# ska-telescope/ska-sdp-distributed-fourier-transform

Hardware: AMD Instinct MI355X
Metric: facet_to_subgrid_contributions_per_s (higher is better)
Workload: dtype complex64 (f32 arithmetic)

## Files before the change

### include/swiftly_hip.h

```cpp
#ifndef SWIFTLY_HIP_H
#define SWIFTLY_HIP_H

#include <stddef.h>
#include <stdint.h>

#ifdef __cplusplus
extern "C" {
#endif

typedef struct swiftly_hip swiftly_hip_t;

enum { SWIFTLY_C64 = 0, SWIFTLY_C128 = 1 };
enum {
    SWIFTLY_OK = 0,
    SWIFTLY_ERR_PARAM = 1,
    SWIFTLY_ERR_UNSUPPORTED = 2,
    SWIFTLY_ERR_HIP = 3
};

const char* swiftly_hip_last_error(void);
int swiftly_hip_version(void);
int swiftly_hip_device_count(void);
const char* swiftly_hip_build_id(void);

// ... 185 lines not shown
                                               const int64_t* sub_off0s, void* g_out, int64_t g_facet_stride,
                                               int64_t g_sub_stride, const int64_t* g_offsets,
                                               const int64_t* g_facet_strides, void* stream);
int swiftly_hip_k3_one_launch(int on);

int swiftly_hip_sum_finish_facets(swiftly_hip_t* h, int dtype, const void* in, int64_t nfacets, int64_t in_facet_stride,
                                  int64_t in_sub_stride, int64_t in_row_stride, const int64_t* facet_off0s,
                                  const int64_t* facet_off1s, void* out, int64_t out_sub_stride, int64_t out_row_stride,
                                  const int64_t* subgrid_off1s, int64_t subgrid_size, const void* mask,
                                  int64_t mask_batch_stride, int64_t nsub, void* stream);

int swiftly_hip_wave_facet_side(swiftly_hip_t* h, int dtype, const void* bands, int64_t rows, int64_t band_row_stride,
                                int64_t band_facet_stride, int64_t nfacets, const int64_t* facet_off0s,
                                int64_t band_start, int64_t band_len, int64_t wave_off1, const int32_t* rowmap,
                                int64_t n_rows, void* q_work, int64_t q_facet_stride, int compute_q, int64_t nsub,
                                const int64_t* sub_off0s, void* g_out, int64_t g_facet_stride, int64_t g_sub_stride,
                                const int64_t* g_offsets, const int64_t* g_facet_strides, void* scratch,
                                int64_t scratch_bytes, void* stream);
int swiftly_hip_wave_subgrid_side(swiftly_hip_t* h, int dtype, const void* g, int64_t nfacets, int64_t g_facet_stride,
                                  int64_t g_sub_stride, const int64_t* facet_off0s, const int64_t* facet_off1s,
                                  int64_t nsub, const int64_t* sub_off0s, const int64_t* sub_off1s, int64_t subgrid_size,
                                  const void* mask0, int64_t mask0_bs, const void* mask1, int64_t mask1_bs,
                                  void* tmp_work, void* out, void* scratch, int64_t scratch_bytes, void* stream);

int swiftly_hip_wave_group_finish_pieces(swiftly_hip_t* h, int dtype, int64_t npieces, const void* const* q,
                                         const int64_t* q_facet_strides, const int32_t* const* rowmaps,
                                         const int64_t* n_rows, const int64_t* first, const int64_t* count,
                                         int64_t nfacets, const int64_t* facet_off0s, const int64_t* facet_off1s,
                                         int64_t nsub, const int64_t* sub_off0s, const int64_t* sub_off1s,
                                         int64_t subgrid_size, const void* mask0, int64_t mask0_bs, const void* mask1,
                                         int64_t mask1_bs, void* t_work, int64_t t_work_elems, void* out, int stages,
                                         void* stream);
int swiftly_hip_group_finish(int on);

int swiftly_hip_finish_axis1_rows(swiftly_hip_t* h, int dtype, const void* bands, int64_t rows, int64_t band_row_stride,
                                  int64_t band_facet_stride, int64_t nfacets, const int64_t* facet_off1s,
                                  int64_t band_start, int64_t band_len, int64_t wave_off1, void* out,
                                  int64_t out_row_stride, int64_t out_facet_stride, void* stream);
int swiftly_hip_wave_subgrid_side_placed(swiftly_hip_t* h, int dtype, const void* g, int64_t nfacets, int64_t g_facet_stride,
                                         int64_t g_sub_stride, const int64_t* facet_off0s, const int64_t* facet_off1s,
                                         int64_t nsub, const int64_t* sub_off0s, const int64_t* sub_off1s,
                                         int64_t subgrid_size, const void* mask0, int64_t mask0_bs, const void* mask1,
                                         int64_t mask1_bs, void* tmp_work, void* out, void* scratch, int64_t scratch_bytes,
                                         void* stream);

int swiftly_hip_prepare_facet_window_rows(swiftly_hip_t* h, int dtype, const void* in, int64_t rows, int64_t facet_size,
                                          int64_t in_row_stride, void* out, int64_t out_row_stride, int64_t facet_off,
                                          int64_t band_start, int64_t band_len, int64_t other_axis_size,
                                          int64_t other_axis_row0, const int32_t* window_starts, int64_t nwindows,
                                          int64_t out_window_stride, void* stream);
int swiftly_hip_split_prepare_facets(swiftly_hip_t* h, int dtype, const void* in, int64_t in_sub_stride,
                                     int64_t in_row_stride, int64_t subgrid_size, int64_t nsub,
                                     const int64_t* subgrid_off1s, int64_t nfacets, const int64_t* facet_off0s,
                                     const int64_t* facet_off1s, void* out, int64_t out_facet_stride,
                                     int64_t out_sub_stride, void* stream);

int swiftly_hip_wave_split_subgrids(swiftly_hip_t* h, int dtype, const void* subgrids, int64_t subgrid_size, int64_t nsub,
                                    const int64_t* subgrid_off0s, const int64_t* subgrid_off1s, int64_t nfacets,
                                    const int64_t* facet_off0s, const int64_t* facet_off1s, void* work,
                                    int64_t work_elems, void* out, int64_t out_facet_stride, int64_t out_sub_stride,
                                    void* stream);

int swiftly_hip_accumulate_facet_columns(swiftly_hip_t* h, int dtype, const void* parts, int64_t part_row_stride,
                                         int64_t nchunks, const int64_t* chunk_offsets,
                                         const int64_t* chunk_facet_strides, const int32_t* row_sources,
                                         int64_t nfacets, const int64_t* facet_off0s, int64_t facet_size,
// ... 51 lines not shown
```

### ska-sdp-distributed-fourier-transform_amd/csrc/group_finish.hip

```cpp
#include "swiftly_groupfinish.h"
#include "swiftly_launch.h"

namespace swf {

template <int LOGM, int LOGX>
static int launch_one_g(const GroupFinishArgs& a, int nbatch, int ngroups, hipStream_t s) {
    using S = GFGeo<LOGM, LOGX>;
    dim3 grid((unsigned)((a.ncols + 15) / 16), (unsigned)nbatch, (unsigned)ngroups);
    return launch_lds<group_finish_kernel<LOGM, LOGX>, S::LDS_BYTES>(grid, dim3(S::NT), s, a);
}

int launch_group_finish(int logm, int logx, const GroupFinishArgs& a, int nbatch, int ngroups, hipStream_t s) {
#define GF_CASE(M, XX) \
    if (logm == M && logx == XX) return launch_one_g<M, XX>(a, nbatch, ngroups, s);
    GF_PAIRS(GF_CASE)
#undef GF_CASE
    return -1;
}

}
```

### ska-sdp-distributed-fourier-transform_amd/csrc/swiftly_abi.hip

```cpp
#include <hip/hip_runtime.h>
#include "swiftly_abi_internal.h"

static thread_local std::string g_err;

int fail(int code, const char* fmt, ...) {
    char buf[512];
    va_list ap;
    va_start(ap, fmt);
    vsnprintf(buf, sizeof buf, fmt, ap);
    va_end(ap);
    g_err = buf;
    return code;
}

int launch_status(int e, const char* what, const char* negative) {
    if (!e) return 0;
    const char* text = (e < 0 && negative) ? negative : hipGetErrorString((hipError_t)e);
    if (what) return fail(SWIFTLY_ERR_HIP, "kernel launch failed (%s): %s", what, text);
    return fail(SWIFTLY_ERR_HIP, "kernel launch failed: %s", text);
}
int radix_launch_status(int e, int Q, const char* pass) {
    if (!e) return 0;
    char what[48]; snprintf(what, sizeof what, "radix-%d %s", Q, pass);
    return launch_status(e, what);
// ... 150 lines not shown
    }
    return n;
}

int swiftly_hip_create(swiftly_hip_t** out, int64_t N, int64_t yN, int64_t xM, double W, const double* pswf,
                       int device) {
    if (!out || !pswf) return fail(SWIFTLY_ERR_PARAM, "null argument");
    *out = nullptr;
    if (const std::string bad = check_sizes(N, yN, xM); !bad.empty()) return fail(SWIFTLY_ERR_PARAM, "%s", bad.c_str());
    int ndev = swiftly_hip_device_count();
    if (ndev <= 0) return fail(SWIFTLY_ERR_HIP, "no HIP device visible: the SwiFTly HIP backend has no CPU fallback");
    if (device < 0 || device >= ndev) return fail(SWIFTLY_ERR_PARAM, "invalid device %d", device);
    DeviceGuard guard(device);
    if (guard.rc) return fail(SWIFTLY_ERR_HIP, "hipSetDevice(%d): %s", device, hipGetErrorString((hipError_t)guard.rc));
    std::lock_guard<std::mutex> init_lock(g_init_mutex);
    if ((int)g_device_inited.size() < ndev) g_device_inited.resize(ndev, 0);
    if (!g_device_inited[device]) {
        int lds = 0;
        if (int rc = set_registered_kernel_attributes(&lds))
            return fail(SWIFTLY_ERR_HIP, "kernel attribute setup failed (%d bytes of LDS): %d", lds, rc);
        hipMemPool_t pool;
        if (hipDeviceGetDefaultMemPool(&pool, device) == hipSuccess) {
            uint64_t keep = UINT64_MAX;
            (void)hipMemPoolSetAttribute(pool, hipMemPoolAttrReleaseThreshold, &keep);
        }
        (void)hipGetLastError();
        g_device_inited[device] = 1;
    }
    swiftly_hip* h = new (std::nothrow) swiftly_hip();
    if (!h) return fail(SWIFTLY_ERR_HIP, "out of host memory");
    static_cast<Sizes&>(*h) = make_sizes(N, yN, xM);
    h->W = W;
    h->device = device;
    if (const char* e = getenv("SWIFTLY_COL_F64")) h->col_f64 = atoi(e) != 0;
    if (const char* e = getenv("SWIFTLY_COL_F64_STAGES")) h->col_f64_stages = atoi(e) & 7;
    std::vector<double> ip(yN);
    std::vector<float> ipf(yN);
    for (int64_t k = 0; k < yN; k++) {
        ip[k] = (k == 0 || pswf[k] == 0.0) ? 0.0 : 1.0 / pswf[k];
        ipf[k] = (float)ip[k];
    }
    const int64_t step = N / xM;
    std::vector<double> fn;
    for (int64_t k = (yN / 2) % step; k < yN; k += step) fn.push_back(pswf[k]);
    if ((int64_t)fn.size() != h->m) {
        delete h;
        return fail(SWIFTLY_ERR_PARAM, "internal: Fn length %zu != contribution size %lld", fn.size(), (long long)(xM * yN / N));
    }
    std::vector<float> fnf(fn.begin(), fn.end());
    int rc = 0;
    if (!rc) rc = upload(h, &h->invp_d, ip);
    if (!rc) rc = upload(h, &h->invp_f, ipf);
    if (!rc) rc = upload(h, &h->fn_d, fn);
    if (!rc) rc = upload(h, &h->fn_f, fnf);
    for (int l : {h->log_yN, h->log_xM, h->log_m})
        if (!rc && l >= 0) {
            rc = make_twiddles(h, l);
            if (!rc && l >= kTwoPassMinLog) rc = make_twiddles(h, l / 2);
            if (!rc && l >= kTwoPassMinLog) rc = make_twiddles(h, l - l / 2);
            if (!rc && l == 15) rc = make_twiddles(h, 14);
            if (!rc && l == 15) rc = make_twiddles(h, 13);
            if (!rc && (l == 16 || l == 14)) rc = make_twiddles(h, l - 1);
        }
    if (!rc && h->log_yN == 15) {
        rc = make_compact_twiddles(h, 14, 5);
        if (!rc) h->win4.twc = compact_twiddles(h, 14, 5);
// ... 1096 lines not shown
```

### ska-sdp-distributed-fourier-transform_amd/csrc/swiftly_abi_internal.h

```cpp
#pragma once

#include <algorithm>
#include <cmath>
#include <cstdarg>
#include <cstdio>
#include <cstdlib>
#include <cstring>
#include <map>
#include <atomic>
#include <mutex>
#include <new>
#include <string>
#include <vector>

#include "../../include/swiftly_hip.h"
#include "swiftly_colpass.h"
#include "swiftly_geometry.h"
#include "swiftly_launch.h"
#include "swiftly_rowpass.h"
#include "swiftly_sumfinish.h"
#include "swiftly_rows.h"
#include "swiftly_rowslong.h"
#include "swiftly_bluestein.h"
#include "swiftly_mixed.h"
// ... 9 lines not shown
              "the complex128 backward band stays inside the double twiddle tables, the complex128 column passes and the long-row kernels");

int fail(int code, const char* fmt, ...);
#define HIP_TRY(expr)                                                                      \
    do {                                                                                   \
        hipError_t e_ = (expr);                                                            \
        if (e_ != hipSuccess) return fail(SWIFTLY_ERR_HIP, "%s: %s", #expr, hipGetErrorString(e_)); \
    } while (0)
int launch_status(int e, const char* what = nullptr, const char* negative = nullptr);
int radix_launch_status(int e, int Q, const char* pass = "pass");

struct ScratchLease {
    void* p = nullptr; bool own = false; hipStream_t st = nullptr;
    int acquire(void* ws, size_t ws_bytes, size_t need, hipStream_t stream, const char* what) {
        own = !(ws && ws_bytes >= need);
        st = stream;
        p = ws;
        if (!own) return 0;
        const hipError_t e = hipMallocAsync(&p, need, st);
        if (e == hipSuccess) return 0;
        own = false;
        return fail(SWIFTLY_ERR_HIP, "%s: %s", what, hipGetErrorString(e));
    }
    int release(int rc) {
        const hipError_t e = own ? hipFreeAsync(p, st) : hipSuccess;
        own = false;
        return (!rc && e != hipSuccess) ? fail(SWIFTLY_ERR_HIP, "hipFreeAsync: %s", hipGetErrorString(e)) : rc;
    }
};

struct swiftly_hip : Sizes {
    double W;
    int device;
    float* invp_f = nullptr;
    double* invp_d = nullptr;
    float* fn_f = nullptr;
    double* fn_d = nullptr;
    std::map<int, cx<float>*> tw_f;
    std::map<int, cx<double>*> tw_d;
    std::map<std::pair<int, int>, cx<float>*> twc_f;
    struct Blu {
        int logL = 0;
        cx<float>* chirp_f = nullptr;
        cx<float>* spec_f = nullptr;
        cx<double>* chirp_d = nullptr;
        cx<double>* spec_d = nullptr;
    };
    std::map<int64_t, Blu> blu;
    struct Mixed {
        int Q = 0, logM = 0;
        cx<float>* tw_f = nullptr;
        cx<double>* tw_d = nullptr;
    };
    std::map<int64_t, Mixed> mixed;
    std::vector<void*> allocs;
    int col_f64 = 0;
    int col_f64_stages = 7;
    hipStream_t chunk_st[2] = {nullptr, nullptr};
    std::mutex chunk_mu;
    std::atomic<void*> ws_plain_pending{nullptr};
    Win4Cache win4;
};

template <typename R>
inline MixedArgs<R> mixed_args(const swiftly_hip::Mixed& mx, int64_t n) {
    MixedArgs<R> X;
// ... 196 lines not shown
```

### ska-sdp-distributed-fourier-transform_amd/csrc/swiftly_abi_pipeline.hip

```cpp
#include "swiftly_abi_internal.h"
#include "swiftly_groupfinish.h"

__global__ void mark_columns_kernel(unsigned char* __restrict__ touched, int m, int rot, int base, int yN, int band_start,
                                    int band_len) {
    const int col = blockIdx.x * blockDim.x + threadIdx.x;
    if (col >= m) return;
    int scol = base + ((col + rot) & (m - 1));
    if (scol >= yN) scol -= yN;
    int d = scol - band_start;
    if (d < 0) d += yN;
    if (d < band_len) touched[d] = 1;
}
template <typename R>
__global__ void zero_untouched_kernel(cx<R>* __restrict__ band, const unsigned char* __restrict__ touched, long long rows,
                                      long long pitch, int band_len) {
    const int d = blockIdx.x * blockDim.x + threadIdx.x;
    if (d >= band_len || touched[d]) return;
    for (long long r = blockIdx.y; r < rows; r += gridDim.y) band[r * pitch + d] = cx<R>{(R)0, (R)0};
}


extern "C" {

int swiftly_hip_sum_finish_rows(swiftly_hip_t* h, int dtype, const void* in, int64_t ngroups, int64_t in_group_stride,
// ... 385 lines not shown
        }
    }
    return 0;
}

static int check_window_pieces(const swiftly_hip_t* h, const char* who, int64_t npieces, const void* const* q,
                               const int64_t* q_facet_strides, const int64_t* n_rows, const int64_t* first,
                               const int64_t* count) {
    if (npieces < 0 || npieces > 2) return fail(SWIFTLY_ERR_PARAM, "%s: 0..2 pieces, got %lld", who, (long long)npieces);
    const int64_t m = h->m;
    int64_t covered = 0;
    for (int64_t i = 0; i < npieces; i++) {
        if (count[i] < 0 || first[i] < 0 || first[i] + count[i] > m || first[i] % 16 || count[i] % 16)
            return fail(SWIFTLY_ERR_PARAM, "%s: piece %lld = [%lld, +%lld) must be multiples of 16 "
                        "inside [0, %lld)", who, (long long)i, (long long)first[i], (long long)count[i], (long long)m);
        if (count[i] && (!q[i] || n_rows[i] <= 0 || n_rows[i] > h->yN || q_facet_strides[i] < n_rows[i] * m))
            return fail(SWIFTLY_ERR_PARAM, "bad row count %lld / facet stride %lld", (long long)n_rows[i], (long long)q_facet_strides[i]);
        covered += count[i];
    }
    if (npieces == 2 && count[0] && count[1] && first[0] < first[1] + count[1] && first[1] < first[0] + count[0])
        return fail(SWIFTLY_ERR_PARAM, "%s: the pieces overlap", who);
    if (covered != m) return fail(SWIFTLY_ERR_PARAM, "%s: the pieces hold %lld of %lld positions", who, (long long)covered, (long long)m);
    return 0;
}

static void window_piece_roles(int64_t m, int64_t npieces, const int64_t* first, const int64_t* count, int* a, int* b) {
    *a = *b = -1;
    for (int64_t i = 0; i < npieces; i++)
        if (count[i]) *(first[i] == 0 && count[i] < m ? b : a) = (int)i;
}

static std::atomic<int> g_k3_one_launch{getenv("SWIFTLY_K3_ONE_LAUNCH") ? atoi(getenv("SWIFTLY_K3_ONE_LAUNCH")) != 0 : 1};
static std::atomic<int> g_group_finish{getenv("SWIFTLY_GROUP_FINISH") ? atoi(getenv("SWIFTLY_GROUP_FINISH")) != 0 : 1};

extern "C" {
int swiftly_hip_k3_one_launch(int on) {
    return on < 0 ? g_k3_one_launch.load() : g_k3_one_launch.exchange(on ? 1 : 0);
}

int swiftly_hip_transform_contributions(swiftly_hip_t* h, int dtype, const void* in, int layout, int64_t in_row_stride,
                                        int64_t in_facet_stride, int64_t in_sub_stride, const int32_t* in_rowmap,
                                        int64_t band_start, int64_t band_len, int64_t nfacets,
                                        const int64_t* facet_off0s, int64_t nsub, const int64_t* subgrid_offs,
                                        void* out, int64_t out_facet_stride, int64_t out_sub_stride, void* stream) {
    if (!h) return fail(SWIFTLY_ERR_PARAM, "null argument");
    DeviceGuard device_guard_(h->device);
    return transform_contributions_impl(h, dtype, in, layout, in_row_stride, in_facet_stride, in_sub_stride, in_rowmap,
                                        band_start, band_len, nfacets, facet_off0s, nsub, subgrid_offs, out,
                                        out_facet_stride, out_sub_stride, nullptr, nullptr, stream);
}

int swiftly_hip_transform_contributions_pieces(swiftly_hip_t* h, int dtype, int64_t npieces, const void* const* q,
                                               const int64_t* q_facet_strides, const int32_t* const* rowmaps,
                                               const int64_t* n_rows, const int64_t* first, const int64_t* count,
                                               int64_t nfacets, const int64_t* facet_off0s, int64_t nsub,
                                               const int64_t* sub_off0s, void* g_out, int64_t g_facet_stride,
                                               int64_t g_sub_stride, const int64_t* g_offsets,
                                               const int64_t* g_facet_strides, void* stream) {
    if (!h || !q || !q_facet_strides || !rowmaps || !n_rows || !first || !count || !g_out || !facet_off0s || !sub_off0s)
        return fail(SWIFTLY_ERR_PARAM, "null argument");
    if (!g_offsets != !g_facet_strides) return fail(SWIFTLY_ERR_PARAM, "g_offsets and g_facet_strides go together");
    if (int rc = check_window_pieces(h, "transform_contributions_pieces", npieces, q, q_facet_strides, n_rows, first, count)) return rc;
    DeviceGuard device_guard_(h->device);
    const int64_t m = h->m;
    int a, b;
    window_piece_roles(m, npieces, first, count, &a, &b);
// ... 245 lines not shown
                                    tmp_work, xM * xA, xA, sub_off1s, subgrid_size, mask1, mask1_bs, nsub, placed, stream);
    if (rc) return rc;
    CallWorkspace call_ws(scratch, scratch ? (size_t)scratch_bytes : 0);
    return swiftly_hip_finish_subgrid_batch(h, dtype, tmp_work, xA, 1, xA, out, 1, xA, 0, subgrid_size, mask0, nsub,
                                            xM * xA, xA * xA, sub_off0s, mask0 ? mask0_bs : 0, stream);
}

int swiftly_hip_wave_subgrid_side(swiftly_hip_t* h, int dtype, const void* g, int64_t nfacets, int64_t g_facet_stride,
                                  int64_t g_sub_stride, const int64_t* facet_off0s, const int64_t* facet_off1s,
                                  int64_t nsub, const int64_t* sub_off0s, const int64_t* sub_off1s, int64_t subgrid_size,
                                  const void* mask0, int64_t mask0_bs, const void* mask1, int64_t mask1_bs,
                                  void* tmp_work, void* out, void* scratch, int64_t scratch_bytes, void* stream) {
    return wave_subgrid_side_impl(h, dtype, g, nfacets, g_facet_stride, g_sub_stride, facet_off0s, facet_off1s, nsub, sub_off0s,
                                  sub_off1s, subgrid_size, mask0, mask0_bs, mask1, mask1_bs, tmp_work, out, scratch, scratch_bytes,
                                  0, stream);
}

int swiftly_hip_wave_subgrid_side_placed(swiftly_hip_t* h, int dtype, const void* g, int64_t nfacets, int64_t g_facet_stride,
                                         int64_t g_sub_stride, const int64_t* facet_off0s, const int64_t* facet_off1s,
                                         int64_t nsub, const int64_t* sub_off0s, const int64_t* sub_off1s,
                                         int64_t subgrid_size, const void* mask0, int64_t mask0_bs, const void* mask1,
                                         int64_t mask1_bs, void* tmp_work, void* out, void* scratch, int64_t scratch_bytes,
                                         void* stream) {
    return wave_subgrid_side_impl(h, dtype, g, nfacets, g_facet_stride, g_sub_stride, facet_off0s, facet_off1s, nsub, sub_off0s,
                                  sub_off1s, subgrid_size, mask0, mask0_bs, mask1, mask1_bs, tmp_work, out, scratch, scratch_bytes,
                                  1, stream);
}


int swiftly_hip_group_finish(int on) {
    return on < 0 ? g_group_finish.load() : g_group_finish.exchange(on ? 1 : 0);
}

int swiftly_hip_wave_group_finish_pieces(swiftly_hip_t* h, int dtype, int64_t npieces, const void* const* q,
                                         const int64_t* q_facet_strides, const int32_t* const* rowmaps,
                                         const int64_t* n_rows, const int64_t* first, const int64_t* count,
                                         int64_t nfacets, const int64_t* facet_off0s, const int64_t* facet_off1s,
                                         int64_t nsub, const int64_t* sub_off0s, const int64_t* sub_off1s,
                                         int64_t subgrid_size, const void* mask0, int64_t mask0_bs, const void* mask1,
                                         int64_t mask1_bs, void* t_work, int64_t t_work_elems, void* out, int stages,
                                         void* stream) {
    if (!h || !q || !q_facet_strides || !rowmaps || !n_rows || !first || !count || !t_work || !facet_off0s || !facet_off1s ||
        !sub_off0s || !sub_off1s || (!out && (stages & 2)))
        return fail(SWIFTLY_ERR_PARAM, "null argument");
    if (stages < 1 || stages > 3) return fail(SWIFTLY_ERR_PARAM, "wave_group_finish_pieces: stages must be 1, 2 or 3");
    CHECK_SUBGRID_SIZE();
    if (nfacets <= 0) return fail(SWIFTLY_ERR_UNSUPPORTED, "wave_group_finish_pieces: 1..%d facets supported", kGroupFinishMaxFacets);
    if (const std::string why = why_not_group_finish(*h, dtype, nfacets); !why.empty())
        return fail(SWIFTLY_ERR_UNSUPPORTED, "wave_group_finish_pieces: %s", why.c_str());
    if (h->col_f64)
        return fail(SWIFTLY_ERR_UNSUPPORTED, "wave_group_finish_pieces: float32 column arithmetic only (column precision is 64)");
    if (int rc = check_window_pieces(h, "wave_group_finish_pieces", npieces, q, q_facet_strides, n_rows, first, count)) return rc;
    if (nsub <= 0) return 0;
    DeviceGuard device_guard_(h->device);
    const int m = (int)h->m, xM = (int)h->xM, xA = (int)subgrid_size, yN = (int)h->yN, ratio = xM / m;
    CHECK_OFFSETS_32(offsets_fit_32(yN, m, yN));

    SumFinishFacetArgs r;
    std::memset(&r, 0, sizeof r);
    fill_facet_groups(r, h, nfacets, facet_off0s, facet_off1s);
    const int ngroups = r.ngroups;
    if (t_work_elems < (int64_t)ngroups * nsub * xM * m)
        return fail(SWIFTLY_ERR_PARAM, "t_work holds %lld elements, %lld needed", (long long)t_work_elems,
                    (long long)((int64_t)ngroups * nsub * xM * m));
    GroupFinishArgs a;
    std::memset(&a, 0, sizeof a);
// ... 17 lines not shown
    a.tw_x = twiddles<float>(h, h->log_xM);
    if (!a.fn || !a.tw_m || !a.tw_x) return fail(SWIFTLY_ERR_HIP, "internal: missing twiddle tables");
    a.mask_bs = mask0 ? mask0_bs : 0;

    for (int g = 0; g < ngroups; g++) {
        r.gstart[g] = g * ratio;
        for (int c = 0; c < ratio; c++) {
            r.fidx[g * ratio + c] = (int)((int64_t)g * nsub * ratio + c);
            r.base0[g * ratio + c] = c * m;
        }
    }
    r.gstart[ngroups] = ngroups * ratio;
    r.nfacets = ngroups * ratio;
    r.in_fs = (long long)m * m; r.in_bs = (long long)xM * m; r.in_rs = m;
    r.out_bs = (long long)xA * xA; r.out_rs = xA;
    r.nrows = xA;
    r.xA = xA;
    fill_group_rounds(r, h);
    r.mask_bs = mask1 ? mask1_bs : 0;
    if (int rc = fill_sum_finish_tables(h, false, &r.fn, &r.tw_m, &r.tw_x, &r.twc_m, &r.twc_x)) return rc;

    static_assert(kGroupFinishMaxBatch == kSumFinishMaxBatch, "one batch loop");
    for (int64_t b0 = 0; b0 < nsub; b0 += kGroupFinishMaxBatch) {
        const int nb = (int)std::min<int64_t>(kGroupFinishMaxBatch, nsub - b0);
        if (stages & 1) {
            a.out = (cx<float>*)t_work + b0 * a.out_bs;
            a.mask = mask0 ? (const float*)mask0 + b0 * mask0_bs : nullptr;
            for (int b = 0; b < nb; b++) {
                const Window w = window_of(*h, sub_off0s[b0 + b]);
                a.lda[b] = w.rot;
                a.ldc[b] = w.base;
                a.st_a[b] = subgrid_in_padded_subgrid(*h, xA, sub_off0s[b0 + b]).a;
            }
            if (int rc = launch_status(launch_group_finish(h->log_m, h->log_xM, a, nb, ngroups, (hipStream_t)stream), "group_finish",
                                       "no instance"))
                return rc;
        }
        if (stages & 2) {
            r.in = (const cx<float>*)t_work + b0 * r.in_bs;
            r.out = (cx<float>*)out + b0 * r.out_bs;
            r.mask = mask1 ? (const float*)mask1 + b0 * mask1_bs : nullptr;
            for (int b = 0; b < nb; b++) r.st_a[b] = subgrid_in_padded_subgrid(*h, xA, sub_off1s[b0 + b]).a;
            if (int rc = launch_status(launch_sum_finish_facets(h->log_m, h->log_xM, r, nb, (hipStream_t)stream))) return rc;
        }
    }
    return 0;
}

int swiftly_hip_accumulate_facet_columns(swiftly_hip_t* h, int dtype, const void* parts, int64_t part_row_stride,
                                         int64_t nchunks, const int64_t* chunk_offsets,
                                         const int64_t* chunk_facet_strides, const int32_t* row_sources,
                                         int64_t nfacets, const int64_t* facet_off0s, int64_t facet_size,
                                         const void* masks, int64_t subgrid_off1, void* bands, int64_t band_row_stride,
                                         int64_t band_facet_stride, int64_t band_start, int64_t band_len,
                                         unsigned char* touched, void* workspace, int64_t workspace_bytes,
                                         void* stream) {
    if (!h || !parts || !bands || !chunk_offsets || !chunk_facet_strides || !row_sources || !facet_off0s)
        return fail(SWIFTLY_ERR_PARAM, "null argument");
    DeviceGuard device_guard_(h->device);
    const bool c128 = dtype == SWIFTLY_C128;
    CHECK_DTYPE();
    CHECK_FACET_SIZE();
    const int yN = (int)h->yN, m = (int)h->m;
    const swiftly_hip::Mixed* mx = nullptr;
    if (h->log_yN < 0) {
        auto it = h->mixed.find(h->yN);
        if (it != h->mixed.end() && it->second.tw_f && !band_is_split(h)) mx = &it->second;
    }
    if (const std::string why = why_not_backward_band(*h, dtype, true); !why.empty())
// ... 112 lines not shown
```

### ska-sdp-distributed-fourier-transform_amd/csrc/swiftly_groupfinish.h

```cpp
#pragma once
#include "swiftly_caps.h"
#include "swiftly_colpass.h"

namespace swf {

constexpr int kGroupFinishMaxBatch = 64;

struct GroupFinishArgs {
    const cx<float>* in_a;
    const cx<float>* in_b;
    long long in_fs_a, in_fs_b;
    const int* rowmap_a;
    const int* rowmap_b;
    unsigned in_pitch;
    int split;
    cx<float>* out;
    long long out_gs, out_bs;
    int yN, xA;
    int ncols;
    int gstart[kGroupFinishMaxFacets + 1];
    int fidx[kGroupFinishMaxFacets];
    int sp0[kGroupFinishMaxFacets];
    int lda[kGroupFinishMaxBatch], ldc[kGroupFinishMaxBatch];
    int st_a[kGroupFinishMaxBatch];
// ... 74 lines not shown
            constexpr int LR = GM::LOGN % GM::LOGP == 0 ? GM::LOGP : GM::LOGN % GM::LOGP, RAD = 1 << LR, NBL = PM / RAD;
            constexpr int slot = (decltype(sI)::value / RAD) + NBL * (decltype(sI)::value % RAD);
            const int ck = e ^ (M >> 1);
            const int kk = (ck - sp) & (M - 1);
            const int p = (kk - (M >> 1) + sp) & (X - 1);
            const int c = p >> LOGM;
            const float w = A.fn[kk];
            static_for<0, RATIO>([&](auto cI) {
                constexpr int cc = decltype(cI)::value;
                const float wc = c == cc ? w : 0.f;
                y[slot + PM * cc].x += v.x * wc;
                y[slot + PM * cc].y += v.y * wc;
            });
        });
        static_for<0, PM>([&](auto vI) { x[decltype(vI)::value] = xn[decltype(vI)::value]; });
    }

    static_for<0, PX>([&](auto vI) { y[decltype(vI)::value].y = -y[decltype(vI)::value].y; });
    cx<float>* __restrict__ out = A.out + (long long)g * A.out_gs + (long long)b * A.out_bs + col;
    const float* __restrict__ mask = A.mask ? A.mask + (long long)b * A.mask_bs : nullptr;
    const int st_a = A.st_a[b];
    const float scale = 1.f / (float)X;
    fft_phases<GX, float, 0>(y, tr, c16, true, smem, A.tw_x, [&](int e, cx<float> v) {
        const int ck = e ^ (X >> 1);
        const int d = (ck + st_a) & (X - 1);
        if (d < A.xA && live) {
            float w = scale;
            if (mask) w *= mask[d];
            cp_store<true>(out + (unsigned)d * (unsigned)A.ncols, cx<float>{v.x * w, -v.y * w});
        }
    });
}

int launch_group_finish(int logm, int logx, const GroupFinishArgs& a, int nbatch, int ngroups, hipStream_t s);

}
```

### ska-sdp-distributed-fourier-transform_amd/ska_sdp_exec_swiftly_amd/_lib.py

```python
import ctypes
import os
from ctypes import POINTER, c_char_p, c_double, c_int, c_int64, c_size_t, c_void_p

_HERE = os.path.dirname(os.path.abspath(__file__))
LIB_PATH = os.path.join(_HERE, os.environ.get("SWIFTLY_HIP_LIB", "libswiftly_hip.so"))

C64, C128 = 0, 1
ERR_PARAM, ERR_UNSUPPORTED, ERR_HIP = 1, 2, 3
(FEATURE_FUSED_SUBGRID, FEATURE_BAND_PIPELINE, FEATURE_BAND_PIPELINE_EXPLICIT, FEATURE_BACKWARD_BAND, FEATURE_SPLIT_BAND,
 FEATURE_WINDOW_ROWS, FEATURE_BACKWARD_BAND_EXPLICIT, FEATURE_SPLIT_PREPARE, FEATURE_REAL_FACETS,
 FEATURE_REAL_FACETS_OUT, FEATURE_GROUP_FINISH) = range(11)
LIMIT_FUSED_FACETS, LIMIT_WINDOW_ROWS_STAGE_COLUMNS, LIMIT_WINDOW_ROWS_WINDOWS = range(3)

_lib = None


class SwiftlyHipError(RuntimeError):
    """HIP runtime / launch failure reported by libswiftly_hip.so"""


def _declare(lib):
    i64, vp = c_int64, c_void_p
    lib.swiftly_hip_last_error.restype = c_char_p
    lib.swiftly_hip_last_error.argtypes = []
# ... 82 lines not shown
    lib.swiftly_hip_prepare_facet_columns.argtypes = [vp, c_int, vp, i64, i64, i64, i64, pi64, i64, i64, i64, vp, i64, i64, vp, vp]
    lib.swiftly_hip_transform_contributions.restype = c_int
    lib.swiftly_hip_transform_contributions.argtypes = [
        vp, c_int, vp, c_int, i64, i64, i64, vp, i64, i64, i64, pi64, i64, pi64, vp, i64, i64, vp,
    ]
    lib.swiftly_hip_sum_finish_facets.restype = c_int
    lib.swiftly_hip_sum_finish_facets.argtypes = [
        vp, c_int, vp, i64, i64, i64, i64, pi64, pi64, vp, i64, i64, pi64, i64, vp, i64, i64, vp,
    ]
    lib.swiftly_hip_wave_facet_side.restype = c_int
    lib.swiftly_hip_wave_facet_side.argtypes = [
        vp, c_int, vp, i64, i64, i64, i64, pi64, i64, i64, i64, vp, i64, vp, i64, c_int, i64, pi64, vp, i64, i64, pi64, pi64,
        vp, i64, vp,
    ]
    lib.swiftly_hip_prepare_facet_columns_waves.restype = c_int
    lib.swiftly_hip_prepare_facet_columns_waves.argtypes = [
        vp, c_int, vp, i64, i64, i64, i64, pi64, i64, i64, i64, pi64, vp, i64, i64, i64, vp, i64, vp, i64, vp,
    ]
    lib.swiftly_hip_prepare_facet_columns_range.restype = c_int
    lib.swiftly_hip_prepare_facet_columns_range.argtypes = [
        vp, c_int, vp, i64, i64, i64, i64, pi64, i64, i64, i64, i64, i64, vp, i64, i64, vp, vp, i64, vp,
    ]
    lib.swiftly_hip_transform_contributions_pieces.restype = c_int
    lib.swiftly_hip_transform_contributions_pieces.argtypes = [
        vp, c_int, i64, POINTER(vp), pi64, POINTER(vp), pi64, pi64, pi64, i64, pi64, i64, pi64, vp, i64, i64, pi64, pi64, vp,
    ]
    lib.swiftly_hip_wave_group_finish_pieces.restype = c_int
    lib.swiftly_hip_wave_group_finish_pieces.argtypes = [
        vp, c_int, i64, POINTER(vp), pi64, POINTER(vp), pi64, pi64, pi64, i64, pi64, pi64, i64, pi64, pi64, i64, vp, i64, vp,
        i64, vp, i64, vp, c_int, vp,
    ]
    lib.swiftly_hip_group_finish.restype = c_int
    lib.swiftly_hip_group_finish.argtypes = [c_int]
    lib.swiftly_hip_wave_subgrid_side.restype = c_int
    lib.swiftly_hip_wave_subgrid_side.argtypes = [
        vp, c_int, vp, i64, i64, i64, pi64, pi64, i64, pi64, pi64, i64, vp, i64, vp, i64, vp, vp, vp, i64, vp,
    ]
    lib.swiftly_hip_wave_subgrid_side_placed.restype = c_int
    lib.swiftly_hip_wave_subgrid_side_placed.argtypes = list(lib.swiftly_hip_wave_subgrid_side.argtypes)
    lib.swiftly_hip_prepare_facet_window_rows.restype = c_int
    lib.swiftly_hip_prepare_facet_window_rows.argtypes = [
        vp, c_int, vp, i64, i64, i64, vp, i64, i64, i64, i64, i64, i64, vp, i64, i64, vp,
    ]
    lib.swiftly_hip_finish_axis1_rows.restype = c_int
    lib.swiftly_hip_finish_axis1_rows.argtypes = [vp, c_int, vp, i64, i64, i64, i64, pi64, i64, i64, i64, vp, i64, i64, vp]
    lib.swiftly_hip_accumulate_facet_columns.restype = c_int
    lib.swiftly_hip_accumulate_facet_columns.argtypes = [
        vp, c_int, vp, i64, i64, pi64, pi64, vp, i64, pi64, i64, vp, i64, vp, i64, i64, i64, i64, vp, vp, i64, vp,
    ]
    lib.swiftly_hip_split_prepare_facets.restype = c_int
    lib.swiftly_hip_split_prepare_facets.argtypes = [vp, c_int, vp, i64, i64, i64, i64, pi64, i64, pi64, pi64, vp, i64, i64, vp]
    lib.swiftly_hip_wave_split_subgrids.restype = c_int
    lib.swiftly_hip_wave_split_subgrids.argtypes = [vp, c_int, vp, i64, i64, pi64, pi64, i64, pi64, pi64, vp, i64, vp, i64, i64, vp]
    lib.swiftly_hip_band_zero_untouched.restype = c_int
    lib.swiftly_hip_band_zero_untouched.argtypes = [vp, c_int, vp, i64, i64, i64, vp, vp]
    lib.swiftly_hip_finish_facet_band.restype = c_int
    lib.swiftly_hip_finish_facet_band.argtypes = [vp, c_int, vp, i64, i64, i64, i64, vp, i64, i64, i64, vp, vp]
    lib.swiftly_hip_finish_facet_band_real.restype = c_int
    lib.swiftly_hip_finish_facet_band_real.argtypes = list(lib.swiftly_hip_finish_facet_band.argtypes)
    src = [c_int, vp, i64, i64, i64]
    for name, args in [
        ("subgrids_from_sources", src + [pi64, pi64, i64, vp, vp, vp, i64, i64, vp]),
        ("check_subgrids_from_sources", src + [pi64, pi64, i64, vp, vp, vp, i64, i64, vp, vp]),
        ("facet_from_sources", src + [i64, i64, vp, vp, vp, i64, vp]),
        ("check_facet_from_sources", src + [i64, i64, vp, vp, vp, i64, vp, vp, vp, vp]),
    ]:
# ... 74 lines not shown
```

Baseline: 135,000.

## Add persistent group-finish kernel with cross-tile prefetch and LDS-cached twiddles

Adds a persistent variant of the group_finish kernel, enabled by default, whose grid is capped at the compute-unit count and which walks tiles in a grid-stride loop. Twiddles, Fn weights and row maps are staged in LDS once per block. While the axis-X FFT and stores of the current tile run, the first input rows of the next tile are prefetched. This is meant to cut launch and tail overhead and hide load latency. In exchange it uses more registers and LDS, and a one-block-per-CU grid may leave the GPU underoccupied.

```diff
diff --git a/include/swiftly_hip.h b/include/swiftly_hip.h
--- a/include/swiftly_hip.h
+++ b/include/swiftly_hip.h
@@ -241,6 +241,7 @@
                                          int64_t mask1_bs, void* t_work, int64_t t_work_elems, void* out, int stages,
                                          void* stream);
 int swiftly_hip_group_finish(int on);
+int swiftly_hip_group_finish_persistent(int n);
 
 int swiftly_hip_finish_axis1_rows(swiftly_hip_t* h, int dtype, const void* bands, int64_t rows, int64_t band_row_stride,
                                   int64_t band_facet_stride, int64_t nfacets, const int64_t* facet_off1s,
diff --git a/ska-sdp-distributed-fourier-transform_amd/csrc/group_finish.hip b/ska-sdp-distributed-fourier-transform_amd/csrc/group_finish.hip
--- a/ska-sdp-distributed-fourier-transform_amd/csrc/group_finish.hip
+++ b/ska-sdp-distributed-fourier-transform_amd/csrc/group_finish.hip
@@ -4,15 +4,21 @@
 namespace swf {
 
 template <int LOGM, int LOGX>
-static int launch_one_g(const GroupFinishArgs& a, int nbatch, int ngroups, hipStream_t s) {
+static int launch_one_g(const GroupFinishArgs& a, int nbatch, int ngroups, int grid_cap, hipStream_t s) {
     using S = GFGeo<LOGM, LOGX>;
-    dim3 grid((unsigned)((a.ncols + 15) / 16), (unsigned)nbatch, (unsigned)ngroups);
-    return launch_lds<group_finish_kernel<LOGM, LOGX>, S::LDS_BYTES>(grid, dim3(S::NT), s, a);
+    const unsigned ntx = (unsigned)((a.ncols + 15) / 16);
+    if (grid_cap <= 0)
+        return launch_lds<group_finish_kernel<LOGM, LOGX>, S::LDS_BYTES>(dim3(ntx, (unsigned)nbatch, (unsigned)ngroups), dim3(S::NT), s,
+                                                                        a);
+    const long long ntiles = (long long)ntx * nbatch * ngroups;
+    if (ntiles <= 0 || ntiles > 0x7fffffff) return (int)hipErrorInvalidValue;
+    const dim3 grid((unsigned)std::min<long long>(ntiles, grid_cap));
+    return launch_lds<group_finish_kernel_persistent<LOGM, LOGX>, GFPersistentLds<LOGM, LOGX>::BYTES>(grid, dim3(S::NT), s, a, nbatch, (int)ntiles);
 }
 
-int launch_group_finish(int logm, int logx, const GroupFinishArgs& a, int nbatch, int ngroups, hipStream_t s) {
+int launch_group_finish(int logm, int logx, const GroupFinishArgs& a, int nbatch, int ngroups, int grid_cap, hipStream_t s) {
 #define GF_CASE(M, XX) \
-    if (logm == M && logx == XX) return launch_one_g<M, XX>(a, nbatch, ngroups, s);
+    if (logm == M && logx == XX) return launch_one_g<M, XX>(a, nbatch, ngroups, grid_cap, s);
     GF_PAIRS(GF_CASE)
 #undef GF_CASE
     return -1;
diff --git a/ska-sdp-distributed-fourier-transform_amd/csrc/swiftly_abi.hip b/ska-sdp-distributed-fourier-transform_amd/csrc/swiftly_abi.hip
--- a/ska-sdp-distributed-fourier-transform_amd/csrc/swiftly_abi.hip
+++ b/ska-sdp-distributed-fourier-transform_amd/csrc/swiftly_abi.hip
@@ -206,6 +206,10 @@
     static_cast<Sizes&>(*h) = make_sizes(N, yN, xM);
     h->W = W;
     h->device = device;
+    if (hipDeviceGetAttribute(&h->cu_count, hipDeviceAttributeMultiprocessorCount, device) != hipSuccess || h->cu_count <= 0) {
+        delete h;
+        return fail(SWIFTLY_ERR_HIP, "cannot query the compute unit count of device %d", device);
+    }
     if (const char* e = getenv("SWIFTLY_COL_F64")) h->col_f64 = atoi(e) != 0;
     if (const char* e = getenv("SWIFTLY_COL_F64_STAGES")) h->col_f64_stages = atoi(e) & 7;
     std::vector<double> ip(yN);
diff --git a/ska-sdp-distributed-fourier-transform_amd/csrc/swiftly_abi_internal.h b/ska-sdp-distributed-fourier-transform_amd/csrc/swiftly_abi_internal.h
--- a/ska-sdp-distributed-fourier-transform_amd/csrc/swiftly_abi_internal.h
+++ b/ska-sdp-distributed-fourier-transform_amd/csrc/swiftly_abi_internal.h
@@ -65,6 +65,7 @@
 struct swiftly_hip : Sizes {
     double W;
     int device;
+    int cu_count = 0;
     float* invp_f = nullptr;
     double* invp_d = nullptr;
     float* fn_f = nullptr;
diff --git a/ska-sdp-distributed-fourier-transform_amd/csrc/swiftly_abi_pipeline.hip b/ska-sdp-distributed-fourier-transform_amd/csrc/swiftly_abi_pipeline.hip
--- a/ska-sdp-distributed-fourier-transform_amd/csrc/swiftly_abi_pipeline.hip
+++ b/ska-sdp-distributed-fourier-transform_amd/csrc/swiftly_abi_pipeline.hip
@@ -441,6 +441,9 @@
 
 static std::atomic<int> g_k3_one_launch{getenv("SWIFTLY_K3_ONE_LAUNCH") ? atoi(getenv("SWIFTLY_K3_ONE_LAUNCH")) != 0 : 1};
 static std::atomic<int> g_group_finish{getenv("SWIFTLY_GROUP_FINISH") ? atoi(getenv("SWIFTLY_GROUP_FINISH")) != 0 : 1};
+static std::atomic<int> g_group_finish_persistent{
+    getenv("SWIFTLY_GROUP_FINISH_PERSISTENT") ? std::max(0, atoi(getenv("SWIFTLY_GROUP_FINISH_PERSISTENT"))) : 1};
+static thread_local int t_group_finish_last_grid = -1;
 
 extern "C" {
 int swiftly_hip_k3_one_launch(int on) {
@@ -752,6 +755,11 @@
     return on < 0 ? g_group_finish.load() : g_group_finish.exchange(on ? 1 : 0);
 }
 
+int swiftly_hip_group_finish_persistent(int n) {
+    if (n == -2) return t_group_finish_last_grid;
+    return n < 0 ? g_group_finish_persistent.load() : g_group_finish_persistent.exchange(n);
+}
+
 int swiftly_hip_wave_group_finish_pieces(swiftly_hip_t* h, int dtype, int64_t npieces, const void* const* q,
                                          const int64_t* q_facet_strides, const int32_t* const* rowmaps,
                                          const int64_t* n_rows, const int64_t* first, const int64_t* count,
@@ -835,9 +843,12 @@
                 a.ldc[b] = w.base;
                 a.st_a[b] = subgrid_in_padded_subgrid(*h, xA, sub_off0s[b0 + b]).a;
             }
-            if (int rc = launch_status(launch_group_finish(h->log_m, h->log_xM, a, nb, ngroups, (hipStream_t)stream), "group_finish",
-                                       "no instance"))
+            const int persistent = g_group_finish_persistent.load();
+            const int grid_cap = persistent == 1 ? h->cu_count : persistent;
+            if (int rc = launch_status(launch_group_finish(h->log_m, h->log_xM, a, nb, ngroups, grid_cap, (hipStream_t)stream),
+                                       "group_finish", "no instance"))
                 return rc;
+            t_group_finish_last_grid = (int)std::min<int64_t>((int64_t)((m + 15) / 16) * nb * ngroups, grid_cap);
         }
         if (stages & 2) {
             r.in = (const cx<float>*)t_work + b0 * r.in_bs;
diff --git a/ska-sdp-distributed-fourier-transform_amd/csrc/swiftly_groupfinish.h b/ska-sdp-distributed-fourier-transform_amd/csrc/swiftly_groupfinish.h
--- a/ska-sdp-distributed-fourier-transform_amd/csrc/swiftly_groupfinish.h
+++ b/ska-sdp-distributed-fourier-transform_amd/csrc/swiftly_groupfinish.h
@@ -130,6 +130,149 @@
     });
 }
 
-int launch_group_finish(int logm, int logx, const GroupFinishArgs& a, int nbatch, int ngroups, hipStream_t s);
-
+template <int LOGM, int LOGX>
+struct GFPersistentLds {
+    static constexpr int M = 1 << LOGM, X = 1 << LOGX;
+    static constexpr size_t TW_X = GFGeo<LOGM, LOGX>::LDS_BYTES, TW_M = TW_X + X * sizeof(cx<float>),
+                            FN = TW_M + M * sizeof(cx<float>), ROWS = FN + M * sizeof(float), BYTES = ROWS + M * sizeof(int);
+};
+
+template <int LOGM, int LOGX>
+__global__ __launch_bounds__((GFGeo<LOGM, LOGX>::NT)) void group_finish_kernel_persistent(const GroupFinishArgs A, const int nbatch,
+                                                                                          const int ntiles) {
+    using S = GFGeo<LOGM, LOGX>;
+    using GM = typename S::GM;
+    using GX = typename S::GX;
+    using L = GFPersistentLds<LOGM, LOGX>;
+    extern __shared__ __attribute__((aligned(16))) unsigned char smem[];
+    constexpr int M = 1 << LOGM, X = 1 << LOGX, T = S::T, PM = GM::P, PX = GX::P, RATIO = X / M, NT = S::NT;
+    static_assert(PX == PM * RATIO, "accumulator slots");
+    static_assert(M <= NT, "one thread per window row");
+    cx<float>* const tw_x = reinterpret_cast<cx<float>*>(smem + L::TW_X);
+    cx<float>* const tw_m = reinterpret_cast<cx<float>*>(smem + L::TW_M);
+    float* const fn = reinterpret_cast<float*>(smem + L::FN);
+    int* const rows = reinterpret_cast<int*>(smem + L::ROWS);
+    int tr = threadIdx.x >> 4, c16 = threadIdx.x & 15;
+    const int ntx = (A.ncols + 15) >> 4;
+
+    auto decode = [&](int t, int& tx, int& b, int& g) {
+        const int q = t / ntx;
+        tx = __builtin_amdgcn_readfirstlane(t - q * ntx);
+        g = __builtin_amdgcn_readfirstlane(q / nbatch);
+        b = __builtin_amdgcn_readfirstlane(q - g * nbatch);
+    };
+    auto window_row = [&](int tx, int b) {
+        const int* __restrict__ rowmap = tx * 16 < A.split ? A.rowmap_b : A.rowmap_a;
+        const int q = (((int)threadIdx.x ^ (M >> 1)) + A.lda[b]) & (M - 1);
+        int idx = q + A.ldc[b];
+        if (idx >= A.yN) idx -= A.yN;
+        return rowmap ? rowmap[idx] : idx;
+    };
+    auto load_rows = [&](cx<float> (&dst)[PM], int n, int tx) {
+        const bool from_b = tx * 16 < A.split;
+        const int col = tx * 16 + c16;
+        const bool live = col < A.ncols;
+        const cx<float>* __restrict__ in =
+            (from_b ? A.in_b : A.in_a) + col + (long long)A.fidx[n] * (from_b ? A.in_fs_b : A.in_fs_a);
+        static_for<0, PM>([&](auto vI) {
+            constexpr int v = decltype(vI)::value;
+            const int row = rows[tr + v * T];
+            cx<float> val = {0.f, 0.f};
+            if (row >= 0 && live) val = cp_load<true>(in + (unsigned)row * A.in_pitch);
+            dst[v] = val;
+        });
+    };
+    auto touch = [](cx<float> (&v)[PM]) {
+        static_for<0, PM>([&](auto vI) {
+            const float re = v[decltype(vI)::value].x, im = v[decltype(vI)::value].y;
+            asm volatile("" ::"v"(re), "v"(im) : "memory");
+        });
+    };
+
+    int t = blockIdx.x, tx, b, g;
+    if (t >= ntiles) return;
+    decode(t, tx, b, g);
+    for (int i = threadIdx.x; i < X; i += NT) tw_x[i] = A.tw_x[i];
+    for (int i = threadIdx.x; i < M; i += NT) {
+        tw_m[i] = A.tw_m[i];
+        fn[i] = A.fn[i];
+    }
+    if (threadIdx.x < M) rows[threadIdx.x] = window_row(tx, b);
+    __syncthreads();
+    cx<float> x[PM], xn[PM];
+    if (A.gstart[g] < A.gstart[g + 1]) load_rows(x, A.gstart[g], tx);
+    touch(x);
+    for (;;) {
+        asm volatile("" : "+v"(tr), "+v"(c16));
+        const int t_next = t + gridDim.x;
+        const bool more = t_next < ntiles;
+        int tx_next = 0, b_next = 0, g_next = 0, row_next = 0;
+        if (more) {
+            decode(t_next, tx_next, b_next, g_next);
+            if (threadIdx.x < M) row_next = window_row(tx_next, b_next);
+        }
+        cx<float> y[PX];
+        static_for<0, PX>([&](auto vI) { y[decltype(vI)::value] = cx<float>{0.f, 0.f}; });
+        const int n_end = A.gstart[g + 1];
+        for (int n = A.gstart[g]; n < n_end; n++) {
+            const int sp = A.sp0[n];
+            if (n + 1 < n_end) load_rows(xn, n + 1, tx);
+            fft_phases<GM, float, 0>(x, tr, c16, true, smem, tw_m, [&](int e, cx<float> v, auto sI) {
+                constexpr int LR = GM::LOGN % GM::LOGP == 0 ? GM::LOGP : GM::LOGN % GM::LOGP, RAD = 1 << LR, NBL = PM / RAD;
+                constexpr int slot = (decltype(sI)::value / RAD) + NBL * (decltype(sI)::value % RAD);
+                const int ck = e ^ (M >> 1);
+                const int kk = (ck - sp) & (M - 1);
+                const int p = (kk - (M >> 1) + sp) & (X - 1);
+                const int c = p >> LOGM;
+                const float w = fn[kk];
+                static_for<0, RATIO>([&](auto cI) {
+                    constexpr int cc = decltype(cI)::value;
+                    const float wc = c == cc ? w : 0.f;
+                    y[slot + PM * cc].x += v.x * wc;
+                    y[slot + PM * cc].y += v.y * wc;
+                });
+            });
+            static_for<0, PM>([&](auto vI) { x[decltype(vI)::value] = xn[decltype(vI)::value]; });
+            touch(x);
+        }
+
+        const int col = tx * 16 + c16;
+        const bool live = col < A.ncols;
+        cx<float>* __restrict__ out = A.out + (long long)g * A.out_gs + (long long)b * A.out_bs + col;
+        const float* __restrict__ mask = A.mask ? A.mask + (long long)b * A.mask_bs : nullptr;
+        const int st_a = A.st_a[b];
+        t = t_next; tx = tx_next; b = b_next; g = g_next;
+        asm volatile("" ::"v"(row_next) : "memory");
+        if (more) {
+            if (threadIdx.x < M) rows[threadIdx.x] = row_next;
+            __syncthreads();
+            if (A.gstart[g] < A.gstart[g + 1]) load_rows(x, A.gstart[g], tx);
+        }
+
+        static_for<0, PX>([&](auto vI) { y[decltype(vI)::value].y = -y[decltype(vI)::value].y; });
+        const float scale = 1.f / (float)X;
+        cx<float> z[PX];
+        int d[PX];
+        fft_phases<GX, float, 0>(y, tr, c16, true, smem, tw_x, [&](int e, cx<float> v, auto sI) {
+            z[decltype(sI)::value] = v;
+            d[decltype(sI)::value] = ((e ^ (X >> 1)) + st_a) & (X - 1);
+        });
+        touch(x);
+        float w[PX];
+        static_for<0, PX>([&](auto sI) { w[decltype(sI)::value] = scale; });
+        if (mask)
+            static_for<0, PX>([&](auto sI) {
+                constexpr int s = decltype(sI)::value;
+                w[s] *= mask[d[s] < A.xA ? d[s] : A.xA - 1];
+            });
+        static_for<0, PX>([&](auto sI) {
+            constexpr int s = decltype(sI)::value;
+            if (d[s] < A.xA && live) cp_store<true>(out + (unsigned)d[s] * (unsigned)A.ncols, cx<float>{z[s].x * w[s], -z[s].y * w[s]});
+        });
+        if (!more) break;
+    }
 }
+
+int launch_group_finish(int logm, int logx, const GroupFinishArgs& a, int nbatch, int ngroups, int grid_cap, hipStream_t s);
+
+}
diff --git a/ska-sdp-distributed-fourier-transform_amd/ska_sdp_exec_swiftly_amd/_lib.py b/ska-sdp-distributed-fourier-transform_amd/ska_sdp_exec_swiftly_amd/_lib.py
--- a/ska-sdp-distributed-fourier-transform_amd/ska_sdp_exec_swiftly_amd/_lib.py
+++ b/ska-sdp-distributed-fourier-transform_amd/ska_sdp_exec_swiftly_amd/_lib.py
@@ -138,6 +138,8 @@
     ]
     lib.swiftly_hip_group_finish.restype = c_int
     lib.swiftly_hip_group_finish.argtypes = [c_int]
+    lib.swiftly_hip_group_finish_persistent.restype = c_int
+    lib.swiftly_hip_group_finish_persistent.argtypes = [c_int]
     lib.swiftly_hip_wave_subgrid_side.restype = c_int
     lib.swiftly_hip_wave_subgrid_side.argtypes = [
         vp, c_int, vp, i64, i64, i64, pi64, pi64, i64, pi64, pi64, i64, vp, i64, vp, i64, vp, vp, vp, i64, vp,
```

After: 136,500, median of 6. Within noise of the previous version (+1.2%).
